# cambyse/po-rrt

Hardware: AMD Instinct MI355X
Metric: RRT node-expansions/sec on map_benchmark.pgm (higher is better)
Workload: dtype f64

## Files before the change

### po_rrt_amd/csrc/porrt_device.hpp

```cpp
#pragma once
#include <hip/hip_runtime.h>
#include <stdint.h>
#include <string>
#include <vector>
#include "../../include/porrt_hip.h"

namespace porrt {

template <int NEV>
struct ScopedEvents {
    hipEvent_t e[NEV];
    ScopedEvents() { for (int i = 0; i < NEV; ++i) e[i] = nullptr; }
    hipError_t create() {
        for (int i = 0; i < NEV; ++i) { const hipError_t r = hipEventCreate(&e[i]); if (r != hipSuccess) return r; }
        return hipSuccess;
    }
    ~ScopedEvents() { for (int i = 0; i < NEV; ++i) if (e[i]) (void)hipEventDestroy(e[i]); }
    ScopedEvents(const ScopedEvents &) = delete;
    ScopedEvents &operator=(const ScopedEvents &) = delete;
};

template <class Launch, class GoingOn>
static int sweep_to_fixpoint(hipStream_t stream, uint32_t *flags, size_t rows, int cur, Launch &&launch, GoingOn &&going_on, const char *who,
                             uint64_t &sweeps, std::string &err) {
// ... 91 lines not shown
#else
#define PORRT_T0() do {} while (0)
#define PORRT_TACC(rc, slot) do {} while (0)
#endif
#ifndef PORRT_TIMING_FROM
#define PORRT_TIMING_FROM 0
#endif
#ifndef PORRT_TIMING_UNTIL
#define PORRT_TIMING_UNTIL 0x7FFFFFFF
#endif
#if defined(PORRT_TIMING) && PORRT_TIMING == 1
#define PORRT_TACC_A(rc, slot) do { if (b >= (uint32_t)PORRT_TIMING_FROM && b < (uint32_t)PORRT_TIMING_UNTIL) PORRT_TACC(rc, slot); else t__0 = wall_clock64(); } while (0)
#define PORRT_TACC_B(rc, slot) do { (void)t__0; } while (0)
#elif defined(PORRT_TIMING)
#define PORRT_TACC_A(rc, slot) do { (void)t__0; } while (0)
#define PORRT_TACC_B(rc, slot) do { if (b >= (uint32_t)PORRT_TIMING_FROM && b < (uint32_t)PORRT_TIMING_UNTIL) PORRT_TACC(rc, slot); else t__0 = wall_clock64(); } while (0)
#else
#define PORRT_TACC_A(rc, slot) do {} while (0)
#define PORRT_TACC_B(rc, slot) do {} while (0)
#endif
#if defined(PORRT_TIMING) && PORRT_TIMING == 3
#undef PORRT_TACC_B
#define PORRT_TACC_B(rc, slot) do { (void)t__0; } while (0)
#define PORRT_TACC_C(rc, slot) PORRT_TACC(rc, slot)
#elif defined(PORRT_TIMING)
#define PORRT_TACC_C(rc, slot) do { (void)t__0; } while (0)
#else
#define PORRT_TACC_C(rc, slot) do {} while (0)
#endif

#if defined(PORRT_TIMING) && PORRT_TIMING == 4
#undef PORRT_TACC_B
#define PORRT_TACC_B(rc, slot) do { (void)t__0; } while (0)
#define PORRT_TACC_H(rc, slot) do { if (b >= (uint32_t)PORRT_TIMING_FROM && b < (uint32_t)PORRT_TIMING_UNTIL) PORRT_TACC(rc, slot); else t__0 = wall_clock64(); } while (0)
#define PORRT_TACC_S(rc, slot) do { if (TeamT::kSize == 64 && b >= (uint32_t)PORRT_TIMING_FROM && b < (uint32_t)PORRT_TIMING_UNTIL) PORRT_TACC(rc, slot); else t__0 = wall_clock64(); } while (0)
#elif defined(PORRT_TIMING)
#define PORRT_TACC_H(rc, slot) do { (void)t__0; } while (0)
#define PORRT_TACC_S(rc, slot) PORRT_TACC_B(rc, slot)
#else
#define PORRT_TACC_H(rc, slot) do {} while (0)
#define PORRT_TACC_S(rc, slot) do {} while (0)
#endif
#if defined(PORRT_TIMING) && PORRT_TIMING == 5
#undef PORRT_TACC_B
#define PORRT_TACC_B(rc, slot) do { (void)t__0; } while (0)
#endif

struct BestCost {
    unsigned long long cost_bits;
    uint32_t final_id, path_len, overflow, pad;
};

typedef float flt2 __attribute__((ext_vector_type(2)));
struct RunConst {
    double *nx, *ny;
    int *rep;
    flt2 *rep_f;
    double bx0, by0, binv_w, binv_h;
    uint32_t *rg_cnt;
    unsigned long long *rg_occ;
    uint32_t *rg_dir;
    double *pg_xy;
    int *pg_id;
    double *pg_d;
    uint32_t *slot_of;
    uint32_t rg_maxp, pg_cap;
    double *distA, *distB;
    int *parent;
    unsigned long long *reachA, *reachB;
    uint8_t *vid;
    uint8_t *final_flag;
    unsigned long long *final_mask;
    uint32_t *n_at;
    unsigned long long *valid_mask;
    Counters *cnt;
    double *sx, *sy;
    uint32_t *sworld;
    const double *inj_xy;
    unsigned long long inj_base, inj_n;
    double *q_x, *q_y;
    double *kq_x, *kq_y;
    int *kq_vid;
    int *q_nn;
    int *q_vid;
    uint32_t *cand_cnt;
    int *cand_id;
    double *cand_val;
    double *cand_xy;
    uint32_t cand_cap;
    uint32_t cand_K;
    const double *rad_T2;
    uint32_t *e_from, *e_to, *e_tv;
    uint32_t e_cap;
    KdRec *kd_rec;
    KdBox *kd_box;
    KdBox *loc_box;
    uint32_t loc_stride;
    KdMove *kd_losers;
    int *pend_new, *pend_pool;
    uint32_t *pend_off, *pend_n, *pend_cur, *pend_state;
    uint32_t pend_cap, pool_cap;
    int *bc_scratch;
    uint32_t bc_cap;
    uint32_t *bc_cursor;
    BestCost *bc_out;
    unsigned long long *kd_hint;
// ... 1 lines not shown
    uint32_t *kd_depth;
    uint32_t *kd_gexit;
    int *loc_cur;
    uint32_t *loc_dcur, *loc_gex, *loc_flags, *g_nd;
    double *g_nd_x, *g_nd_y;
    KdBox *g_nd_box;
    int *g_id;
    double *g_x, *g_y;
    uint32_t g_cap;
    uint32_t *g_snap;
    double gp_x, gp_y;
    const uint8_t *cls;
    const uint32_t *sat;
    const uint8_t *clr;
    uint32_t W, H;
    double low0, low1, ppm;
    int domain, has_grid;
    int n_validities;
    unsigned long long validities[65];
    unsigned long long all_worlds;
    int goal_kind;
    uint32_t G;
    double gcx[64], gcy[64];
    unsigned long long gmask[64];
    double g_l1;
    double w2g_x[64], w2g_y[64];
    double zone_x, zone_y, visibility;
    double s_low0, s_low1, s_up0, s_up1;
    double max_step;
    int mode;
    uint16_t *perm;
    double *ssx, *ssy;
    double *bq_x, *bq_y;
    uint16_t *bq_k;
    double *t2_at;
    uint32_t tile_R;
    uint32_t part_stride;
    uint32_t q_stride;
    double start_x, start_y;
    unsigned long long root_reach;
    int root_vid;
    unsigned long long rng_st_lo, rng_st_hi, rng_inc_lo, rng_inc_hi;
    struct PcgJump *jump;
    RunConst *self;
    uint32_t *zero0;
    unsigned long long zero_words;
    uint32_t *sched_i0, *sched_nb;
    uint32_t sched_min, sched_max, sched_K, sched_steps;
    uint32_t sched_max_nodes;
    uint32_t cand_par3;
    uint32_t hint_max;
    uint32_t kd_lazy;
};

#define GPTR(T) T __attribute__((address_space(1))) *
template <class T>
__device__ __forceinline__ GPTR(T) as_global(T *p) { return (GPTR(T))(uintptr_t)p; }
template <class T>
__device__ __forceinline__ GPTR(const T) as_global(const T *p) { return (GPTR(const T))(uintptr_t)p; }
template <class T>
__device__ __forceinline__ T g_atomic_add(GPTR(T) p, T v) { return __hip_atomic_fetch_add(p, v, __ATOMIC_RELAXED, __HIP_MEMORY_SCOPE_AGENT); }
template <class T>
__device__ __forceinline__ T g_atomic_or(GPTR(T) p, T v) { return __hip_atomic_fetch_or(p, v, __ATOMIC_RELAXED, __HIP_MEMORY_SCOPE_AGENT); }
template <class T>
__device__ __forceinline__ T g_atomic_min(GPTR(T) p, T v) { return __hip_atomic_fetch_min(p, v, __ATOMIC_RELAXED, __HIP_MEMORY_SCOPE_AGENT); }

__device__ __forceinline__ uint32_t uni(uint32_t v) { return (uint32_t)__builtin_amdgcn_readfirstlane((int)v); }
__device__ __forceinline__ double uni_d(double v) {
    const unsigned long long b = (unsigned long long)__double_as_longlong(v);
    const unsigned long long lo = uni((uint32_t)b), hi = uni((uint32_t)(b >> 32));
    return __longlong_as_double((long long)(lo | (hi << 32)));
}

#ifndef PORRT_RC_SCALAR
#define PORRT_RC_SCALAR 1
#endif
__device__ __forceinline__ const RunConst &rc_const(const RunConst *p) {
#if PORRT_RC_SCALAR
    const uintptr_t a = (uintptr_t)p;
    const uintptr_t u = (uintptr_t)uni((uint32_t)a) | ((uintptr_t)uni((uint32_t)(a >> 32)) << 32);
    return *(const RunConst *)(const RunConst __attribute__((address_space(4))) *)u;
#else
    return *p;
#endif
}
__device__ __forceinline__ const RunConst &rc_const(const RunConst &rc) { return rc_const(&rc); }

__device__ __forceinline__ uint32_t row_nb(const RunConst &rc, uint32_t b, uint32_t nb_arg) {
    return rc.sched_nb ? ((GPTR(const uint32_t))(uintptr_t)rc.sched_nb)[b] : nb_arg;
}
__device__ __forceinline__ uint32_t row_i0(const RunConst &rc, uint32_t b, uint32_t i0_arg) {
    return rc.sched_i0 ? ((GPTR(const uint32_t))(uintptr_t)rc.sched_i0)[b] : i0_arg;
}


__device__ __forceinline__ uint32_t q_off(const RunConst &rc, uint32_t b) { return (b & 1u) * rc.q_stride; }
__device__ __forceinline__ uint32_t cand_slot(const RunConst &rc, uint32_t b) { return rc.cand_par3 ? b % 3u : (b & 1u); }
__device__ __forceinline__ size_t cand_off(const RunConst &rc, uint32_t b, uint32_t k) { return ((size_t)cand_slot(rc, b) * rc.cand_K + k) * rc.cand_cap; }
__device__ __forceinline__ uint32_t cand_cnt_at(const RunConst &rc, uint32_t b, uint32_t k) { return cand_slot(rc, b) * rc.cand_K + k; }
__device__ __forceinline__ size_t cand_val_off(const RunConst &rc, uint32_t b, uint32_t k) {
    return rc.cand_par3 ? ((size_t)cand_slot(rc, b) * rc.cand_K + k) * rc.cand_cap : (size_t)k * rc.cand_cap;
}
__device__ __forceinline__ uint32_t cand_count(const RunConst &rc, uint32_t b, uint32_t k) {
    const uint32_t c = as_global(rc.cand_cnt)[cand_cnt_at(rc, b, k)];
    return c < rc.cand_cap ? c : rc.cand_cap;
}
__device__ __forceinline__ unsigned long long f64_bits(double d) { return (unsigned long long)__double_as_longlong(d); }

__device__ __forceinline__ uint32_t f64_as_u32(double v) {
    if (!(v == v)) return 0u;
    if (v <= 0.0) return 0u;
    if (v >= 4294967295.0) return 4294967295u;
    return (uint32_t)v;
}

__device__ __forceinline__ void to_pixel(const RunConst &rc, double x, double y, uint32_t &i, uint32_t &j) {
    double t = (y - rc.low1) * rc.ppm;
    i = f64_as_u32((double)(rc.H - 1) - t);
    j = f64_as_u32((x - rc.low0) * rc.ppm);
}

__device__ __forceinline__ double dist2(double ax, double ay, double bx, double by) {
    double dx = bx - ax, dy = by - ay;
    double xx = dx * dx, yy = dy * dy;
    return xx + yy;
}

__device__ __forceinline__ void wave_first_min(double &value, uint32_t &pos) {
    constexpr uint32_t kNone = 0xFFFFFFFFu;
    for (uint32_t s = 32; s >= 1; s >>= 1) {
        const double oc = __shfl_xor(value, (int)s);
        const uint32_t op = (uint32_t)__shfl_xor((int)pos, (int)s);
        if (op != kNone && (pos == kNone || oc < value || (oc == value && op < pos))) { value = oc; pos = op; }
    }
}

__device__ __forceinline__ void oct_to(int o, int x, int y, int &ox, int &oy) {
    switch (o) {
    case 0: ox = x; oy = y; break;
// ... 77 lines not shown
    const int fb = (o == 1 || o == 6) ? 1 : ((o == 2 || o == 5) ? -1 : 0);
    const int fc = (o == 1 || o == 2) ? 1 : ((o == 5 || o == 6) ? -1 : 0);
    const int fd = (o == 0 || o == 3) ? 1 : ((o == 4 || o == 7) ? -1 : 0);
    constexpr int kRayChunk = Grid::kRayChunk;
    for (int x = sx, y = sy; x <= ex;) {
        int c[kRayChunk];
        const int n = ex - x + 1 < kRayChunk ? ex - x + 1 : kRayChunk;
#pragma unroll
        for (int u = 0; u < kRayChunk; ++u) {
            c[u] = CLS_FREE;
            if (u < n) {
                const int pi = fa * x + fb * y, pj = fc * x + fd * y;
                c[u] = grid.at((uint32_t)pi, (uint32_t)pj);
                if (e >= 0) { y += 1; e -= ddx; }
                e += ddy;
                ++x;
            }
        }
#pragma unroll
        for (int u = 0; u < kRayChunk; ++u) {
            if (u >= n) break;
            if (rc.domain == 0) {
                if (c[u] == CLS_HIGH0) return CLS_HIGH;
                worst = c[u] > worst ? c[u] : worst;
            } else if (c[u] != CLS_FREE) {
                if (c[u] == CLS_HIGH || c[u] == CLS_HIGH0) return CLS_HIGH;
                if (c[u] == CLS_BAD) { *err |= ERR_RASTER; return CLS_HIGH; }
                if (worst >= CLS_ZONE && worst != c[u]) { *err |= ERR_RASTER; return CLS_HIGH; }
                worst = c[u];
            }
        }
    }
    return worst;
}
template <class Grid>
__device__ __forceinline__ int traversed_class(const RunConst &rc, const Grid &grid, double ax, double ay, double bx, double by, uint32_t *err) {
    uint32_t ai, aj, bi, bj;
    to_pixel(rc, ax, ay, ai, aj);
    to_pixel(rc, bx, by, bi, bj);
    return traversed_class_px(rc, grid, ai, aj, bi, bj, err);
}

__device__ __forceinline__ bool segment_in_clearance(uint32_t ai, uint32_t aj, uint32_t bi, uint32_t bj, uint32_t clr_b) {
    const uint32_t di = ai > bi ? ai - bi : bi - ai, dj = aj > bj ? aj - bj : bj - aj;
    return (di > dj ? di : dj) < clr_b;
}

__device__ __forceinline__ int state_class(const RunConst &rc, double x, double y, uint32_t *err) {
    uint32_t i, j;
    to_pixel(rc, x, y, i, j);
    if (i >= rc.H || j >= rc.W) { *err |= ERR_RASTER; return CLS_HIGH; }
    int c = as_global(rc.cls)[i * rc.W + j];
    if (c == CLS_BAD) { *err |= ERR_RASTER; return CLS_HIGH; }
    return c == CLS_HIGH0 ? CLS_HIGH : c;
}

__device__ __forceinline__ int class_to_validity(const RunConst &rc, int cls) {
    if (cls == CLS_FREE) return rc.n_validities - 1;
    if (cls >= CLS_ZONE) return cls - CLS_ZONE;
    return -1;
}

template <class Grid>
__device__ bool goal_hit(const RunConst &rc, const Grid &grid, double x, double y, unsigned long long &mask, uint32_t *err) {
    if (rc.goal_kind == 1) {
        for (uint32_t g = 0; g < rc.G; ++g) {
            double d = fabs(rc.gcx[g] - x);
            d += fabs(rc.gcy[g] - y);
            if (d < rc.g_l1) { mask = rc.gmask[g]; return true; }
        }
        return false;
    }
    if (rc.goal_kind == 2) {
        double D = sqrt(dist2(x, y, rc.zone_x, rc.zone_y));
        if (D < rc.visibility) {
            int c = traversed_class(rc, grid, x, y, rc.zone_x, rc.zone_y, err);
            if (c != CLS_HIGH) { mask = 1ull; return true; }
        }
    }
    return false;
}

typedef unsigned __int128 u128;
__device__ __forceinline__ u128 mk128(unsigned long long lo, unsigned long long hi) { return ((u128)hi << 64) | lo; }

struct PcgJump {
    unsigned long long mult_lo[64], mult_hi[64], plus_lo[64], plus_hi[64];
};

__device__ __forceinline__ unsigned long long pcg_output(u128 s) {
    uint32_t rot = (uint32_t)(s >> 122);
    unsigned long long xsl = (unsigned long long)(s >> 64) ^ (unsigned long long)s;
    return (xsl >> rot) | (xsl << ((64 - rot) & 63));
}

__device__ __forceinline__ double gen_range_once(unsigned long long r, double low, double high, bool *retry) {
    double v12 = __longlong_as_double((long long)((r >> 12) | 0x3FF0000000000000ull));
    double v01 = v12 - 1.0;
    double scale = high - low;
    double prod = v01 * scale;
    double res = prod + low;
    if (!(res < high)) *retry = true;
    return res;
}

__global__ void k_gen_samples(const RunConst *__restrict__ rcp, const PcgJump *__restrict__ jt, unsigned long long it0,
// ... 560 lines not shown
        as_global(rc.pg_id)[(size_t)page * kPage + (slot % kPage)] = (int)nid;
        as_global(rc.slot_of)[nid] = page * kPage + (slot % kPage);
        if (!GROUP || rc.q_stride) {
            as_global(rc.nx)[nid] = x[q];
            as_global(rc.ny)[nid] = y[q];
        }
    }
#pragma unroll
    for (uint32_t h = 0; h < RPT; ++h) {
        const uint32_t r = tid + h * T;
        if (r < kRegions) rg_new[r] = s_old[r] + s_add[r];
    }
    if (tid < kOccWords) {
        unsigned long long w = 0;
        for (uint32_t i = 0; i < 64u; ++i) {
            const uint32_t r = tid * 64u + i;
            if (r < kRegions && s_old[r] + s_add[r] > 0u) w |= 1ull << i;
        }
        as_global(rc.rg_occ)[((b + 1u) & 1u) * kOccWords + tid] = w;
    }
    if (tid == 0) { as_global(rc.t2_at)[b + 1] = t2_next; rc.cnt->n_pages += s_misc[0]; }
}

__device__ __forceinline__ uint32_t rank_before(const RunConst &rc, uint32_t b, uint32_t vwords, uint32_t k) {
    uint32_t r = 0;
    auto vm = as_global(rc.valid_mask) + (size_t)b * vwords;
    for (uint32_t w = 0; w < (k >> 6); ++w) r += __popcll(vm[w]);
    r += __popcll(vm[k >> 6] & ((1ull << (k & 63u)) - 1ull));
    return r;
}
template <int CTRL>
__device__ __forceinline__ uint32_t dpp_u32(uint32_t v) { return (uint32_t)__builtin_amdgcn_update_dpp((int)v, (int)v, CTRL, 0xF, 0xF, false); }
template <int CTRL>
__device__ __forceinline__ double dpp_f64(double v) {
    const unsigned long long b = (unsigned long long)__double_as_longlong(v);
    const unsigned long long lo = dpp_u32<CTRL>((uint32_t)b), hi = dpp_u32<CTRL>((uint32_t)(b >> 32));
    return __longlong_as_double((long long)(lo | (hi << 32)));
}
constexpr int kDppRowRor = 0x120;
constexpr int kDppRowBcast = 0x150;
#ifndef PORRT_DPP
#define PORRT_DPP 1
#endif

__device__ __forceinline__ uint32_t rank_before_lanes(const RunConst &rc, uint32_t b, uint32_t vwords, uint32_t k, uint32_t lane, uint32_t stride) {
    auto vm = as_global(rc.valid_mask) + (size_t)b * vwords;
    const uint32_t wk = k >> 6;
    uint32_t r = 0;
    for (uint32_t w0 = 0; w0 <= wk; w0 += stride) {
        const uint32_t w = w0 + lane;
        unsigned long long v = w <= wk ? vm[w] : 0ull;
        if (w == wk) v &= (1ull << (k & 63u)) - 1ull;
        r += (uint32_t)__popcll(v);
    }
    if (PORRT_DPP && stride == 16u) {
        r += dpp_u32<kDppRowRor + 8>(r); r += dpp_u32<kDppRowRor + 4>(r); r += dpp_u32<kDppRowRor + 2>(r); r += dpp_u32<kDppRowRor + 1>(r);
        return r;
    }
    for (uint32_t off = stride >> 1; off > 0; off >>= 1) r += (uint32_t)__shfl_xor((int)r, (int)off);
    return r;
}

__device__ __forceinline__ TileGrid load_tile(const RunConst &rc, uint8_t *tile, double px, double py, uint32_t lane, uint32_t stride) {
    TileGrid g;
    g.lds = tile; g.glob = rc.cls; g.W = rc.W; g.TW = 2u * rc.tile_R + 1u;
    uint32_t ci, cj;
    to_pixel(rc, px, py, ci, cj);
    g.oi = (int)ci - (int)rc.tile_R;
    g.oj = (int)cj - (int)rc.tile_R;
    const uint32_t n = g.TW * g.TW;
    for (uint32_t t = lane; t < n; t += stride) {
        const uint32_t ri = t / g.TW, rj = t - ri * g.TW;
        const int i = g.oi + (int)ri, j = g.oj + (int)rj;
        uint8_t c = CLS_BAD;
        if (i >= 0 && j >= 0 && (uint32_t)i < rc.H && (uint32_t)j < rc.W) c = as_global(rc.cls)[(uint32_t)i * rc.W + (uint32_t)j];
        tile[t] = c;
    }
    return g;
}

template <class T>
__device__ __forceinline__ T wave_min_u(T v) {
    for (int off = 32; off > 0; off >>= 1) {
        T o = __shfl_xor(v, off);
        v = o < v ? o : v;
    }
    return v;
}
__device__ __forceinline__ uint32_t wave_sum(uint32_t v) {
    for (int off = 32; off > 0; off >>= 1) v += __shfl_xor(v, off);
    return v;
}
__device__ __forceinline__ unsigned long long wave_or(unsigned long long v) {
    for (int off = 32; off > 0; off >>= 1) v |= __shfl_xor(v, off);
    return v;
}

__device__ __forceinline__ bool kd_left(double x, double y, double wx, double wy, uint32_t depth) {
    return (depth & 1u) ? (y < wy) : (x < wx);
}

__device__ bool kd_preorder_less(const RunConst &rc, int u, int v) {
    const uint32_t gu = as_global(rc.kd_gexit)[u], gv = as_global(rc.kd_gexit)[v];
    const bool ou = gu & kOnG, ov = gv & kOnG;
    const uint32_t iu = gu & ~kOnG, iv = gv & ~kOnG;
    if (ou && ov) return iu < iv;
// ... 2097 lines not shown
```

### po_rrt_amd/csrc/porrt_group.hpp

```cpp
#pragma once
#include "porrt_device.hpp"
#include "porrt_span.hpp"

namespace porrt {


template <int GL, int R, bool WITHD, class Visit>
__device__ __forceinline__ void gscan_disc(const RunConst &rc, uint32_t b, const GTeam<GL> &tm, double qx, double qy, double rho, uint32_t N, Visit visit,
                                           uint32_t skip_region = 0xFFFFFFFFu) {
    const uint32_t gl = tm.gl;
    int cx0, cy0, cx1, cy1;
    rep_cell(rc, qx - rho, qy - rho, kRG, cx0, cy0);
    rep_cell(rc, qx + rho, qy + rho, kRG, cx1, cy1);
    const uint32_t x0 = (uint32_t)cx0, y0 = (uint32_t)cy0;
    const uint32_t w = (uint32_t)(cx1 - cx0 + 1), nreg = w * (uint32_t)(cy1 - cy0 + 1);
    constexpr int U = (int)kPage / GL;
    if (nreg * 16u > N) {
#if !PORRT_PAGE_LOADS
        auto gx = as_global(rc.nx), gy = as_global(rc.ny), gdA = as_global(rc.distA);
#endif
        for (uint32_t j0 = 0; j0 < N; j0 += (uint32_t)(U * GL)) {
            double x[U], y[U], d[U];
#pragma unroll
            for (int u = 0; u < U; ++u) {
                const uint32_t j = j0 + (uint32_t)(GL * u) + gl;
#if PORRT_PAGE_LOADS
                const uint32_t o = (j < N ? j : 0u) * 8u;
                x[u] = g_at(rc.nx, o);
                y[u] = g_at(rc.ny, o);
                d[u] = WITHD ? g_at(rc.distA, o) : 0.0;
#else
                x[u] = gx[j < N ? j : 0u];
                y[u] = gy[j < N ? j : 0u];
                d[u] = WITHD ? gdA[j < N ? j : 0u] : 0.0;
#endif
            }
#pragma unroll
            for (int u = 0; u < U; ++u)
                if (j0 + (uint32_t)(GL * u) < N) visit(x[u], y[u], d[u], (int)(j0 + (uint32_t)(GL * u) + gl), j0 + (uint32_t)(GL * u) + gl < N);
        }
        return;
    }
    auto gcnt = as_global(rc.rg_cnt) + (b & 1u) * kRegions;
    auto gdir = as_global(rc.rg_dir);
#if PORRT_PAGE_LOADS
    const PageBuf pb = page_buf(rc);
#else
    auto gxy = as_global(reinterpret_cast<const dbl2 *>(rc.pg_xy));
    auto gid = as_global(rc.pg_id);
    auto gpd = as_global(rc.pg_d);
#endif
    for (uint32_t r0 = 0; r0 < nreg; r0 += (uint32_t)GL) {
        const uint32_t r = r0 + gl;
        uint32_t reg = 0, cnt = 0;
        if (r < nreg) {
            const uint32_t ry = r / w;
            reg = (y0 + ry) * kRG + x0 + (r - ry * w);
            cnt = reg == skip_region ? 0u : gcnt[reg];
        }
        uint32_t page = reg;
        for (uint32_t lvl = 0;; ++lvl) {
            const uint32_t have = cnt > lvl * kPage ? cnt - lvl * kPage : 0u;
            unsigned long long m = tm.ballot(have > 0u);
            if (!m) break;
            uint32_t page_next = 0;
            if (have > kPage) page_next = gdir[(size_t)reg * rc.rg_maxp + lvl + 1u];
            while (m) {
                uint32_t pg[R], pc[R];
#pragma unroll
                for (int q = 0; q < R; ++q) {
                    pg[q] = 0; pc[q] = 0;
                    if (m) {
                        const int l = (int)__builtin_ctzll(m);
                        m &= m - 1;
                        pg[q] = tm.shfl(page, l);
                        const uint32_t h = tm.shfl(have, l);
                        pc[q] = h < kPage ? h : kPage;
                    }
                }
                dbl2 v[R][U];
                double d[R][U];
                int id[R][U];
#pragma unroll
                for (int q = 0; q < R; ++q)
#pragma unroll
                    for (int u = 0; u < U; ++u) {
                        const uint32_t sl = (uint32_t)(u * GL) + gl;
                        const bool ld = sl < pc[q];
#if PORRT_PAGE_LOADS
                        const uint32_t at = ld ? pg[q] * kPage + sl : kNoSlot;
                        v[q][u] = page_xy(pb, at);
                        id[q][u] = page_id(pb, at);
                        d[q][u] = WITHD ? page_d(pb, at) : 0.0;
#else
                        v[q][u] = ld ? gxy[(size_t)pg[q] * kPage + sl] : dbl2{0.0, 0.0};
                        id[q][u] = ld ? gid[(size_t)pg[q] * kPage + sl] : -1;
                        d[q][u] = (WITHD && ld) ? gpd[(size_t)pg[q] * kPage + sl] : 0.0;
#endif
                    }
#if PORRT_PAGE_LOADS
                __atomic_signal_fence(__ATOMIC_SEQ_CST);
#endif
#pragma unroll
                for (int q = 0; q < R; ++q)
#pragma unroll
                    for (int u = 0; u < U; ++u)
                        if ((uint32_t)(u * GL) < pc[q]) visit(v[q][u].x, v[q][u].y, d[q][u], id[q][u], (uint32_t)(u * GL) + gl < pc[q]);
            }
            page = page_next;
        }
    }
}
// ... 390 lines not shown
#pragma unroll
        for (int u = 0; u < U; ++u) {
            if (!(via[u] >= 0.0) || f64_bits(via[u]) != f64_bits(dB[u])) continue;
#if PORRT_PAGE_LOADS
            auto gpar = g_ptr(rc.parent, (uint32_t)j[u] * 4u);
#else
            auto gpar = as_global(rc.parent) + j[u];
#endif
            int old = *gpar;
            while (old < N || id[u] < old) {
                int expect = old;
                if (__hip_atomic_compare_exchange_strong(gpar, &expect, id[u], __ATOMIC_RELAXED, __ATOMIC_RELAXED, __HIP_MEMORY_SCOPE_AGENT)) break;
                old = expect;
            }
#if PORRT_PAGE_LOADS
            *g_ptr(rc.distA, (uint32_t)j[u] * 8u) = via[u];
            *g_ptr(rc.pg_d, g_at(rc.slot_of, (uint32_t)j[u] * 4u) * 8u) = via[u];
#else
            gdA[j[u]] = via[u];
            gpd[gso[j[u]]] = via[u];
#endif
        }
    }
}

#ifndef PORRT_NN2_WAVES
#define PORRT_NN2_WAVES 5
#endif
template <int GL, int WV = 4>
__global__ __launch_bounds__(WV * 64) __attribute__((amdgpu_waves_per_eu(PORRT_NN2_WAVES, 8))) void k_nn2(const RunConst *__restrict__ rcp, uint32_t b, uint32_t i0, uint32_t nb, uint32_t vwords, uint32_t cb,
                                             uint32_t cnb, uint32_t cflat) {
    static_assert(GL == 16 || GL == 32 || GL == 64, "group size");
    constexpr uint32_t SPB = (uint32_t)WV * 64u / GL;
    uint32_t bx = blockIdx.x, by = blockIdx.y;
    xcd_swizzle(bx, by);
    const RunConst &rc = rc_const(rcp + by);
    GTeam<GL> tm;
    tm.gl = threadIdx.x % GL;
    tm.base = (threadIdx.x & 63u) - tm.gl;
    const uint32_t near_blocks = (nb + SPB - 1u) / SPB;
    if (bx >= near_blocks) {
        if (cflat) {
            PORRT_T0();
            commit_flat_span<(uint32_t)WV * 64u>(rc, cb, vwords, cnb, bx - near_blocks);
            PORRT_TACC_A(rc, 4);
            return;
        }
        const uint32_t ck = (bx - near_blocks) * SPB + threadIdx.x / GL;
        PORRT_T0();
        if (ck < cnb && ck < row_nb(rc, cb, cnb)) commit_rrt_sample(rc, cb, vwords, ck, tm.gl, GL);
        PORRT_TACC_A(rc, 4);
        return;
    }
    const uint32_t slot = bx * SPB + threadIdx.x / GL;
    if (slot >= row_nb(rc, b, nb)) return;
    PORRT_T0();
    const size_t so = (size_t)b * rc.part_stride + slot;
    const uint32_t k = as_global(rc.perm)[so];
    const uint32_t N = as_global(rc.n_at)[b];
    const double sqx = as_global(rc.ssx)[so], sqy = as_global(rc.ssy)[so];
    (void)i0;
    int nn = -1;
    double fx = 0.0, fy = 0.0;
    bool easy = false;
    const double lim = 0.7 * rc.max_step, t2b = as_global(rc.t2_at)[b];
    const double lim2 = lim * lim < t2b ? lim * lim : t2b;
    uint32_t err = 0;
    int cls_own = CLS_FREE;
    if (rc.has_grid) cls_own = state_class(rc, sqx, sqy, &err);
    const double perr = 1.3e-7 * (fabs(sqx) + fabs(sqy) + 2.0 * lim);
    const double limf = lim - perr, limf2 = limf > 0.0 ? (limf * limf < t2b ? limf * limf : t2b * (1.0 - 1e-6)) : -1.0;
    (void)lim2;
    for (int l = 0; l < 2 && !easy; ++l) {
        int cx, cy;
        const int G = rep_dim(l);
        rep_cell(rc, sqx, sqy, G, cx, cy);
        bool near = false;
        if (tm.gl < 9u) {
            const int x = cx + (int)(tm.gl % 3u) - 1, y = cy + (int)(tm.gl / 3u) - 1;
            if (x >= 0 && y >= 0 && x < G && y < G) {
                const flt2 pf = as_global(rc.rep_f)[rep_off(l) + y * G + x];
                near = dist2((double)pf.x, (double)pf.y, sqx, sqy) <= limf2;
            }
        }
        easy = tm.ballot(near) != 0ull;
    }
    PORRT_TACC_A(rc, 0);
    if (!easy) group_nn<GL>(rc, b, tm, N, sqx, sqy, nn, fx, fy);
    PORRT_TACC_A(rc, 1);
    double tx = sqx, ty = sqy;
    if (!easy) {
        double step = fabs(tx - fx);
        step += fabs(ty - fy);
        if (step > rc.max_step) {
            const double lambda = rc.max_step / step;
            double ux = (tx - fx) * lambda, uy = (ty - fy) * lambda;
            tx = fx + ux;
            ty = fy + uy;
        }
    }
    bool valid = true;
    if (rc.has_grid) {
        int cls = cls_own;
        if (tx != sqx || ty != sqy) { err = 0; cls = state_class(rc, tx, ty, &err); }
        valid = cls == CLS_FREE && !err;
    }
    PORRT_TACC_A(rc, 2);
    if (tm.gl == 0) {
        as_global(rc.q_x)[k] = tx;
        as_global(rc.q_y)[k] = ty;
        const size_t o2 = (size_t)b * rc.part_stride + k;
        as_global(rc.kq_x)[o2] = tx; as_global(rc.kq_y)[o2] = ty; as_global(rc.kq_vid)[o2] = valid ? 0 : -1;
        as_global(rc.q_nn)[k] = nn;
        int qv = valid ? 0 : -1;
        if (valid && rc.goal_kind != 0 && tx == rc.gp_x && ty == rc.gp_y) {
            const uint32_t slot = atomicAdd(&rc.cnt->clone_n, 1u);
            if (slot < 64u) { rc.cnt->clone_k[slot] = k; qv = 1; }
        }
        as_global(rc.q_vid)[k] = qv;
        as_global(rc.bq_x)[slot] = tx; as_global(rc.bq_y)[slot] = ty; as_global(rc.bq_k)[slot] = qv == 0 ? (uint16_t)k : (uint16_t)0xFFFFu;
        if (valid) atomicOr(&rc.valid_mask[(size_t)b * vwords + (k >> 6)], 1ull << (k & 63u));
        if (err) atomicOr(&rc.cnt->err, err);
    }
}

__host__ __device__ inline size_t conn2_lds_bytes(uint32_t GL) {
    (void)GL;
    return (64u / 16u) * kHitBytes;
}
static_assert(kInsertLds <= kFileLds && kGTrackLds <= kFileLds, "the filing's one-round-trip form is the largest of the riders' scratch areas");
__host__ __device__ inline size_t conn2_riders_lds_bytes() { return kFileLds; }
__host__ __device__ inline size_t conn2_wg4_lds_bytes(uint32_t GL) {
    const size_t a = 4u * conn2_lds_bytes(GL);
    static_assert(kGTrackLds <= 4u * (64u / 16u) * kHitBytes, "g_track_step uses the same bytes");
    static_assert(kFileLds <= 4u * (64u / 16u) * kHitBytes, "file_step_fast uses the same bytes");
    return a > kInsertLds ? a : kInsertLds;
}

__device__ __forceinline__ void rider_file(const RunConst &rc, uint32_t b, uint32_t nb, uint32_t vwords, uint8_t *lds, uint32_t fast) {
    if (fast && nb <= 4u * 256u) file_step_fast<256u, 4u, true>(rc, b, nb, vwords, lds);
    else insert_step_pages<1>(rc, b, nb, vwords, lds);
}
__device__ __forceinline__ void rider_gtrack(const RunConst &rc, uint32_t b, uint32_t nb, uint32_t vwords, uint8_t *lds, uint32_t fast) {
    if (fast) g_track_step<2>(rc, b, nb, vwords, lds);
    else g_track_step<1>(rc, b, nb, vwords, lds);
}
#if defined(PORRT_TIMING) && PORRT_TIMING == 5
#define RIDERS_T0() const unsigned long long rt__0 = wall_clock64(); const uint32_t rt__w = b < 8u ? 0u : ((rc.cnt->g_first_dup[0] & rc.cnt->g_first_dup[1]) != 0xFFFFFFFFu ? 2u : 1u)
#define RIDERS_MARK(role)                                                                                          \
    do {                                                                                                           \
        __syncthreads();                                                                                           \
        if (threadIdx.x == 0) { atomicAdd(&rc.cnt->tim[3u * (role) + rt__w], wall_clock64() - rt__0); if ((role) == 0u) atomicAdd(&rc.cnt->tim[9u + rt__w], 1ull); } \
    } while (0)
#else
#define RIDERS_T0() do {} while (0)
#define RIDERS_MARK(role) do {} while (0)
#endif

template <int GL>
__device__ __attribute__((noinline)) int group_nn_call(const RunConst &rc_arg, uint32_t b, uint32_t gl, uint32_t base, uint32_t N, double px, double py) {
// ... 155 lines not shown
#else
    uint32_t &err = err_out;
#endif
    const uint32_t lane = threadIdx.x & 63u;
    constexpr uint32_t kWaveHits = (64u / (uint32_t)GL) * (kLdsHits * (uint32_t)(GL / 16));
    Team<1> tw;
    tw.scr_d = nullptr; tw.scr_i = nullptr; tw.wave = 0; tw.lane = lane;
    TableGrid grid;
    grid.p = rc.cls; grid.W = rc.W;
    const uint32_t cap = rc.cand_cap;
    const MemHits Mh = mem_hits(rc, b, kh);
    PORRT_T0();
    if (toth <= kWaveHits) {
        LdsHits Wl;
        Wl.hx = (LdsPtr<double>)wb;
        Wl.hy = Wl.hx + kWaveHits;
        Wl.hd = Wl.hy + kWaveHits;
        Wl.hid = (LdsPtr<int>)(Wl.hd + kWaveHits);
        Wl.out_id = Mh.out_id; Wl.out_val = Mh.out_val; Wl.out_cnt = Mh.out_cnt; Wl.out_cap = Mh.out_cap;
        for (uint32_t a0 = 0; a0 < toth; a0 += 256u) {
            int jd[4];
            dbl2 v[4];
            double d[4];
#pragma unroll
            for (uint32_t u = 0; u < 4u; ++u) {
                const uint32_t a = a0 + u * 64u + lane;
                jd[u] = a < toth ? Mh.sid[a] : 0;
                v[u] = a < toth ? Mh.sxy[a] : dbl2{0.0, 0.0};
                d[u] = a < toth ? Mh.sd[a] : 0.0;
            }
#pragma unroll
            for (uint32_t u = 0; u < 4u; ++u) {
                const uint32_t a = a0 + u * 64u + lane;
                if (a < toth) { Wl.hid[a] = jd[u]; Wl.hx[a] = v[u].x; Wl.hy[a] = v[u].y; Wl.hd[a] = d[u]; }
            }
        }
        __builtin_amdgcn_wave_barrier();
        PORRT_TACC_H(rc, 0);
        connect_rrt_sample(rc, tw, Wl, grid, b, kh, idh, pxh, pyh, toth, err, nullptr, 0, clrh, [&]() { return wave_nn(rc, b, N, pxh, pyh); });
        __builtin_amdgcn_wave_barrier();
        PORRT_TACC_H(rc, 3);
    } else {
        connect_rrt_sample(rc, tw, Mh, grid, b, kh, idh, pxh, pyh, toth < cap ? toth : cap, err, nullptr, 0, clrh,
                           [&]() { return wave_nn(rc, b, N, pxh, pyh); });
    }
#if PORRT_PAGE_LOADS
    if (err) err_out |= err;
#endif
}

#ifndef PORRT_CONN2_WAVES
#define PORRT_CONN2_WAVES 4
#endif
template <int GL>
__device__ __forceinline__ void conn2_wave(const RunConst &rc, uint32_t b, uint32_t vwords, uint32_t N, double T2, uint32_t k, double px, double py, uint8_t *wl) {
    const uint32_t lane = threadIdx.x & 63u;
    GTeam<GL> tm;
    tm.gl = threadIdx.x % GL;
    tm.base = lane - tm.gl;
    const bool act = k != 0xFFFFu;
    uint32_t err = 0;
    PORRT_T0();
    uint32_t id = 0, tot = 0;
    int clr_b = 0;
    bool heavy = false;
    const uint32_t cap = rc.cand_cap;
    TableGrid grid;
    grid.p = rc.cls; grid.W = rc.W;
    if (act) {
        id = N + rank_before_lanes(rc, b, vwords, k, tm.gl, (uint32_t)GL);
        if (rc.has_grid) {
            uint32_t bi, bj;
            to_pixel(rc, px, py, bi, bj);
            if (bi < rc.H && bj < rc.W) clr_b = as_global(rc.clr)[bi * rc.W + bj];
        }
        constexpr uint32_t kHits = kLdsHits * (uint32_t)(GL / 16);
        uint8_t *hb = wl + (lane / (uint32_t)GL) * (kHits * 28u);
        LdsHits L;
        L.hx = (LdsPtr<double>)hb;
        L.hy = L.hx + kHits;
        L.hd = L.hy + kHits;
        L.hid = (LdsPtr<int>)(L.hd + kHits);
        const MemHits M = mem_hits(rc, b, k);
        L.out_id = M.out_id; L.out_val = M.out_val; L.out_cnt = M.out_cnt; L.out_cap = M.out_cap;
        PORRT_TACC_B(rc, 0);
        gscan_disc<GL, 1, true>(rc, b, tm, px, py, disc_radius(T2, px, py), N, [&](double x, double y, double dA, int jd, bool ok) {
            const bool in = ok && dist2(x, y, px, py) <= T2;
            const unsigned long long hm = tm.ballot(in);
            const uint32_t pos = tot + (uint32_t)__popcll(hm & ((1ull << tm.gl) - 1ull));
            if (in) {
                if (pos < kHits) { L.hid[pos] = jd; L.hx[pos] = x; L.hy[pos] = y; L.hd[pos] = dA; }
                else if (pos < cap) { M.sid[pos] = jd; dbl2 v; v.x = x; v.y = y; M.sxy[pos] = v; M.sd[pos] = dA; }
                else err |= (uint32_t)ERR_CAND_OVERFLOW;
            }
            tot += (uint32_t)__popcll(hm);
        });
        __builtin_amdgcn_wave_barrier();
        PORRT_TACC_B(rc, 1);
        if (tot <= kHits) {
            connect_rrt_sample(rc, tm, L, grid, b, k, id, px, py, tot, err, nullptr, 0, clr_b,
                               [&]() { return group_nn_call<GL>(rc, b, tm.gl, tm.base, N, px, py); });
            PORRT_TACC_B(rc, 2);
        } else {
            heavy = true;
            if (tm.gl == 0) atomicAdd(&rc.cnt->n_heavy, 1u);
            for (uint32_t a = tm.gl; a < kHits; a += (uint32_t)GL) {
                M.sid[a] = L.hid[a];
                dbl2 v;
                v.x = L.hx[a]; v.y = L.hy[a];
                M.sxy[a] = v;
                M.sd[a] = L.hd[a];
            }
        }
    }
    unsigned long long hv = __ballot(heavy && tm.gl == 0);
    if (hv) {
        __builtin_amdgcn_s_waitcnt(0x0F70);
        __builtin_amdgcn_wave_barrier();
        while (hv) {
            const int l = (int)__builtin_ctzll(hv);
            hv &= hv - 1;
            const uint32_t kh = uni((uint32_t)__shfl((int)k, l)), idh = uni((uint32_t)__shfl((int)id, l)), toth = uni((uint32_t)__shfl((int)tot, l));
            const int clrh = (int)uni((uint32_t)__shfl(clr_b, l));
            const double pxh = uni_d(__shfl(px, l)), pyh = uni_d(__shfl(py, l));
            heavy_sample_wave<GL>(rc, b, N, kh, idh, toth, clrh, pxh, pyh, wl, err);
        }
        PORRT_TACC_B(rc, 3);
    }
    if (err) atomicOr(&rc.cnt->err, err);
}

template <int GL>
__global__ __launch_bounds__(64) __attribute__((amdgpu_waves_per_eu(PORRT_CONN2_WAVES, 8))) void k_conn2(const RunConst *__restrict__ rcp, uint32_t b, uint32_t nb, uint32_t vwords) {
    static_assert(GL == 16 || GL == 32 || GL == 64, "group size");
    constexpr uint32_t SPB = 64u / GL;
    extern __shared__ __attribute__((aligned(16))) uint8_t lds_dyn[];
    uint32_t bx = blockIdx.x, by = blockIdx.y;
    xcd_swizzle(bx, by);
    const RunConst &rc = rc_const(rcp + by);
    nb = row_nb(rc, b, nb);
    const uint32_t slot = bx * SPB + threadIdx.x / GL;
    if (bx * SPB >= nb) return;
    const uint32_t N = as_global(rc.n_at)[b];
    const double T2 = as_global(rc.t2_at)[b];
    uint32_t k = 0xFFFFu;
    double px = 0.0, py = 0.0;
    if (slot < nb) { k = as_global(rc.bq_k)[slot]; px = as_global(rc.bq_x)[slot]; py = as_global(rc.bq_y)[slot]; }
    conn2_wave<GL>(rc, b, vwords, N, T2, k, px, py, lds_dyn);
}

__global__ __launch_bounds__(256) __attribute__((amdgpu_waves_per_eu(PORRT_CONN2_WAVES, 8))) void k_conn2_riders(const RunConst *__restrict__ rcp, uint32_t b, uint32_t nb, uint32_t vwords, uint32_t lazy,
                                                                                                                  uint32_t fast) {
    extern __shared__ __attribute__((aligned(16))) uint8_t lds_dyn[];
    const RunConst &rc = rc_const(rcp + blockIdx.y);
    const uint32_t role = blockIdx.x;
    nb = row_nb(rc, b, nb);
    if (nb == 0) return;
    RIDERS_T0();
    if (role == 0) rider_file(rc, b, nb, vwords, lds_dyn, fast);
    else if (lazy && role == 2u) rider_gtrack(rc, b, nb, vwords, lds_dyn, fast);
    else clone_workgroup(rc, b, vwords, as_global(rc.n_at)[b], as_global(rc.t2_at)[b], fast);
    RIDERS_MARK(role);
}

template <int GL>
__global__ __launch_bounds__(256) __attribute__((amdgpu_waves_per_eu(PORRT_CONN2_WAVES, 8))) void k_conn2_wg4(const RunConst *__restrict__ rcp, uint32_t b, uint32_t nb, uint32_t vwords, uint32_t lazy, uint32_t fast) {
    static_assert(GL == 16 || GL == 32 || GL == 64, "group size");
    constexpr uint32_t SPB = 256u / GL;
    extern __shared__ __attribute__((aligned(16))) uint8_t lds_dyn[];
    uint32_t bx = blockIdx.x, by = blockIdx.y;
    const uint32_t ns = lazy ? 3u : 2u;
    const uint32_t role = xcd_swizzle_roles(bx, by, ns);
    const RunConst &rc = rc_const(rcp + by);
    nb = row_nb(rc, b, nb);
    if (nb == 0) return;
    if (role == 0) { rider_file(rc, b, nb, vwords, lds_dyn, fast); return; }
    if (lazy && role == 2u) { rider_gtrack(rc, b, nb, vwords, lds_dyn, fast); return; }
    const uint32_t slot = bx * SPB + threadIdx.x / GL;
    const uint32_t N = as_global(rc.n_at)[b];
    const double T2 = as_global(rc.t2_at)[b];
    uint32_t k = 0xFFFFu;
    double px = 0.0, py = 0.0;
    if (role == ns && slot < nb) { k = as_global(rc.bq_k)[slot]; px = as_global(rc.bq_x)[slot]; py = as_global(rc.bq_y)[slot]; }
    if (role == 1) { clone_workgroup(rc, b, vwords, N, T2, fast); return; }
    conn2_wave<GL>(rc, b, vwords, N, T2, k, px, py, lds_dyn + (threadIdx.x >> 6) * conn2_lds_bytes(GL));
}

template <int GL>
__global__ __launch_bounds__(256) void k_commit2(const RunConst *__restrict__ rcp, uint32_t b, uint32_t nb, uint32_t vwords) {
    const RunConst &rc = rc_const(rcp + blockIdx.y);
    const uint32_t k = (blockIdx.x * 256u + threadIdx.x) / GL;
    if (k < nb && k < row_nb(rc, b, nb)) commit_rrt_sample(rc, b, vwords, k, threadIdx.x % GL, GL);
}
__global__ __launch_bounds__(256) __attribute__((amdgpu_waves_per_eu(8, 8))) void k_commit_flat(const RunConst *__restrict__ rcp, uint32_t b, uint32_t nb, uint32_t vwords) {
    commit_flat_span<256u>(rc_const(rcp + blockIdx.y), b, vwords, nb, blockIdx.x);
}

}
```

Baseline: 351.7 million.

## Reorder RunConst fields and hoist scalar loads to cut memory round trips

Reorders the RunConst struct so fields used by the nearest-neighbour and connect kernels sit together, and pins them into scalar registers with inline-asm holds so they arrive in a few batched scalar loads. In the nearest-neighbour step, the own-cell class lookup is split into an issue half and a finish half, overlapping it with the first rep-grid probe. In the connect wave, the valid-mask words and clearance byte are loaded early and the rank computation is deferred into a callback inside the disc scan, so those loads overlap the scan's first loads. This adds struct-layout coupling and more register pressure, and relies on compiler-barrier tricks that could change scheduling unpredictably.

```diff
diff --git a/po_rrt_amd/csrc/porrt_device.hpp b/po_rrt_amd/csrc/porrt_device.hpp
--- a/po_rrt_amd/csrc/porrt_device.hpp
+++ b/po_rrt_amd/csrc/porrt_device.hpp
@@ -167,6 +167,123 @@
 };
 
 typedef float flt2 __attribute__((ext_vector_type(2)));
+#ifndef PORRT_STEP_TRIPS
+#define PORRT_STEP_TRIPS 1
+#endif
+#ifndef PORRT_STEP_TRIPS_NN2
+#define PORRT_STEP_TRIPS_NN2 PORRT_STEP_TRIPS
+#endif
+#ifndef PORRT_STEP_TRIPS_CONN2
+#define PORRT_STEP_TRIPS_CONN2 PORRT_STEP_TRIPS
+#endif
+#if PORRT_STEP_TRIPS
+struct RunConst {
+    uint32_t *sched_nb, *sched_i0;
+    uint32_t *n_at;
+    double *t2_at;
+    uint16_t *perm;
+    double *ssx, *ssy;
+    uint32_t part_stride, q_stride;
+    double max_step;
+    int has_grid, domain;
+    uint32_t W, H;
+    double low0, low1, ppm;
+    const uint8_t *cls;
+    const uint8_t *clr;
+    double bx0, by0, binv_w, binv_h;
+    flt2 *rep_f;
+    int *rep;
+    uint32_t *rg_cnt;
+    unsigned long long *rg_occ;
+    uint32_t *rg_dir;
+    double *pg_xy;
+    int *pg_id;
+    double *pg_d;
+    uint32_t rg_maxp, pg_cap;
+    uint32_t *slot_of;
+    double *nx, *ny;
+    uint16_t *bq_k;
+    double *bq_x, *bq_y;
+    unsigned long long *valid_mask;
+    double *distA, *distB;
+    int *parent;
+    Counters *cnt;
+    uint32_t *cand_cnt;
+    int *cand_id;
+    double *cand_val;
+    double *cand_xy;
+    uint32_t cand_cap, cand_K;
+    uint32_t cand_par3, kd_lazy;
+    double *q_x, *q_y;
+    int *q_nn;
+    int *q_vid;
+    double *kq_x, *kq_y;
+    int *kq_vid;
+    int goal_kind;
+    uint32_t G;
+    double gp_x, gp_y;
+    double g_l1;
+    uint8_t *final_flag;
+    unsigned long long *final_mask;
+    const uint32_t *sat;
+    double zone_x, zone_y, visibility;
+    KdRec *kd_rec;
+    int *kd_up;
+    uint32_t *kd_depth;
+    uint32_t *kd_gexit;
+    int *pend_new, *pend_pool;
+    uint32_t *pend_off, *pend_n, *pend_cur, *pend_state;
+    uint32_t pend_cap, pool_cap;
+    double *g_x, *g_y;
+    int *g_id;
+    uint32_t *g_nd;
+    double *g_nd_x, *g_nd_y;
+    KdBox *g_nd_box;
+    uint32_t g_cap, tile_R;
+    const double *rad_T2;
+    unsigned long long *reachA, *reachB;
+    uint8_t *vid;
+    double *sx, *sy;
+    uint32_t *sworld;
+    const double *inj_xy;
+    unsigned long long inj_base, inj_n;
+    uint32_t *e_from, *e_to, *e_tv;
+    uint32_t e_cap;
+    uint32_t loc_stride;
+    KdBox *kd_box;
+    KdBox *loc_box;
+    KdMove *kd_losers;
+    int *bc_scratch;
+    uint32_t *bc_cursor;
+    BestCost *bc_out;
+    uint32_t bc_cap;
+    int mode;
+    unsigned long long *kd_hint;
+    int *loc_cur;
+    uint32_t *loc_dcur, *loc_gex, *loc_flags;
+    uint32_t *g_snap;
+    int n_validities;
+    int root_vid;
+    unsigned long long all_worlds;
+    double s_low0, s_low1, s_up0, s_up1;
+    double start_x, start_y;
+    unsigned long long root_reach;
+    unsigned long long rng_st_lo, rng_st_hi, rng_inc_lo, rng_inc_hi;
+    struct PcgJump *jump;
+    RunConst *self;
+    uint32_t *zero0;
+    unsigned long long zero_words;
+    uint32_t sched_min, sched_max, sched_K, sched_steps;
+    uint32_t sched_max_nodes;
+    uint32_t hint_max;
+    unsigned long long validities[65];
+    double gcx[64], gcy[64];
+    unsigned long long gmask[64];
+    double w2g_x[64], w2g_y[64];
+    unsigned long long pad_[6];
+};
+static_assert(sizeof(RunConst) % 64 == 0, "a row of an array of rows starts on a cache line");
+#else
 struct RunConst {
     double *nx, *ny;
     int *rep;
@@ -274,6 +391,7 @@
     uint32_t hint_max;
     uint32_t kd_lazy;
 };
+#endif
 
 #define GPTR(T) T __attribute__((address_space(1))) *
 template <class T>
@@ -307,6 +425,49 @@
 #endif
 }
 __device__ __forceinline__ const RunConst &rc_const(const RunConst &rc) { return rc_const(&rc); }
+
+template <class T>
+__device__ __forceinline__ auto rc_bits(T v) {
+    static_assert(sizeof(T) == 4 || sizeof(T) == 8, "a field of one or two registers");
+    if constexpr (sizeof(T) == 8) return __builtin_bit_cast(unsigned long long, v);
+    else return __builtin_bit_cast(uint32_t, v);
+}
+#define PORRT_HS1(a) "s"(::porrt::rc_bits(a))
+#define PORRT_HS2(a, ...) PORRT_HS1(a), PORRT_HS1(__VA_ARGS__)
+#define PORRT_HS3(a, ...) PORRT_HS1(a), PORRT_HS2(__VA_ARGS__)
+#define PORRT_HS4(a, ...) PORRT_HS1(a), PORRT_HS3(__VA_ARGS__)
+#define PORRT_HS5(a, ...) PORRT_HS1(a), PORRT_HS4(__VA_ARGS__)
+#define PORRT_HS6(a, ...) PORRT_HS1(a), PORRT_HS5(__VA_ARGS__)
+#define PORRT_HS7(a, ...) PORRT_HS1(a), PORRT_HS6(__VA_ARGS__)
+#define PORRT_HS8(a, ...) PORRT_HS1(a), PORRT_HS7(__VA_ARGS__)
+#define PORRT_HS9(a, ...) PORRT_HS1(a), PORRT_HS8(__VA_ARGS__)
+#define PORRT_HS10(a, ...) PORRT_HS1(a), PORRT_HS9(__VA_ARGS__)
+#define PORRT_HS11(a, ...) PORRT_HS1(a), PORRT_HS10(__VA_ARGS__)
+#define PORRT_HS12(a, ...) PORRT_HS1(a), PORRT_HS11(__VA_ARGS__)
+#define PORRT_HS13(a, ...) PORRT_HS1(a), PORRT_HS12(__VA_ARGS__)
+#define PORRT_HS14(a, ...) PORRT_HS1(a), PORRT_HS13(__VA_ARGS__)
+#define PORRT_HS15(a, ...) PORRT_HS1(a), PORRT_HS14(__VA_ARGS__)
+#define PORRT_HS16(a, ...) PORRT_HS1(a), PORRT_HS15(__VA_ARGS__)
+#define PORRT_HS17(a, ...) PORRT_HS1(a), PORRT_HS16(__VA_ARGS__)
+#define PORRT_HS18(a, ...) PORRT_HS1(a), PORRT_HS17(__VA_ARGS__)
+#define PORRT_HS19(a, ...) PORRT_HS1(a), PORRT_HS18(__VA_ARGS__)
+#define PORRT_HS20(a, ...) PORRT_HS1(a), PORRT_HS19(__VA_ARGS__)
+#define PORRT_HS21(a, ...) PORRT_HS1(a), PORRT_HS20(__VA_ARGS__)
+#define PORRT_HS22(a, ...) PORRT_HS1(a), PORRT_HS21(__VA_ARGS__)
+#define PORRT_HS23(a, ...) PORRT_HS1(a), PORRT_HS22(__VA_ARGS__)
+#define PORRT_HS24(a, ...) PORRT_HS1(a), PORRT_HS23(__VA_ARGS__)
+#define PORRT_HS25(a, ...) PORRT_HS1(a), PORRT_HS24(__VA_ARGS__)
+#define PORRT_HS26(a, ...) PORRT_HS1(a), PORRT_HS25(__VA_ARGS__)
+#define PORRT_HS27(a, ...) PORRT_HS1(a), PORRT_HS26(__VA_ARGS__)
+#define PORRT_HS28(a, ...) PORRT_HS1(a), PORRT_HS27(__VA_ARGS__)
+#define PORRT_HS_PICK(a1, a2, a3, a4, a5, a6, a7, a8, a9, a10, a11, a12, a13, a14, a15, a16, a17, a18, a19, a20, a21, a22, a23, a24, a25, a26, a27, a28, N, ...) \
+    PORRT_HS##N
+#if PORRT_STEP_TRIPS && PORRT_RC_SCALAR
+#define RC_HOLD(key, ...)                                                                                                                         \
+    asm("" : "+s"(key) : PORRT_HS_PICK(__VA_ARGS__, 28, 27, 26, 25, 24, 23, 22, 21, 20, 19, 18, 17, 16, 15, 14, 13, 12, 11, 10, 9, 8, 7, 6, 5, 4, 3, 2, 1)(__VA_ARGS__))
+#else
+#define RC_HOLD(key, ...) do {} while (0)
+#endif
 
 __device__ __forceinline__ uint32_t row_nb(const RunConst &rc, uint32_t b, uint32_t nb_arg) {
     return rc.sched_nb ? ((GPTR(const uint32_t))(uintptr_t)rc.sched_nb)[b] : nb_arg;
@@ -490,6 +651,16 @@
     if (i >= rc.H || j >= rc.W) { *err |= ERR_RASTER; return CLS_HIGH; }
     int c = as_global(rc.cls)[i * rc.W + j];
     if (c == CLS_BAD) { *err |= ERR_RASTER; return CLS_HIGH; }
+    return c == CLS_HIGH0 ? CLS_HIGH : c;
+}
+__device__ __forceinline__ int state_class_issue(const RunConst &rc, double x, double y, bool &inside) {
+    uint32_t i, j;
+    to_pixel(rc, x, y, i, j);
+    inside = i < rc.H && j < rc.W;
+    return as_global(rc.cls)[inside ? i * rc.W + j : 0u];
+}
+__device__ __forceinline__ int state_class_finish(int c, bool inside, uint32_t *err) {
+    if (!inside || c == CLS_BAD) { *err |= ERR_RASTER; return CLS_HIGH; }
     return c == CLS_HIGH0 ? CLS_HIGH : c;
 }
 
@@ -1156,6 +1327,25 @@
         unsigned long long v = w <= wk ? vm[w] : 0ull;
         if (w == wk) v &= (1ull << (k & 63u)) - 1ull;
         r += (uint32_t)__popcll(v);
+    }
+    if (PORRT_DPP && stride == 16u) {
+        r += dpp_u32<kDppRowRor + 8>(r); r += dpp_u32<kDppRowRor + 4>(r); r += dpp_u32<kDppRowRor + 2>(r); r += dpp_u32<kDppRowRor + 1>(r);
+        return r;
+    }
+    for (uint32_t off = stride >> 1; off > 0; off >>= 1) r += (uint32_t)__shfl_xor((int)r, (int)off);
+    return r;
+}
+
+template <uint32_t NW>
+__device__ __forceinline__ uint32_t rank_of_lane_words(const unsigned long long (&v)[NW], uint32_t k, uint32_t lane, uint32_t stride) {
+    const uint32_t wk = k >> 6;
+    uint32_t r = 0;
+#pragma unroll
+    for (uint32_t u = 0; u < NW; ++u) {
+        const uint32_t w = u * stride + lane;
+        unsigned long long x = w <= wk ? v[u] : 0ull;
+        if (w == wk) x &= (1ull << (k & 63u)) - 1ull;
+        r += (uint32_t)__popcll(x);
     }
     if (PORRT_DPP && stride == 16u) {
         r += dpp_u32<kDppRowRor + 8>(r); r += dpp_u32<kDppRowRor + 4>(r); r += dpp_u32<kDppRowRor + 2>(r); r += dpp_u32<kDppRowRor + 1>(r);
diff --git a/po_rrt_amd/csrc/porrt_group.hpp b/po_rrt_amd/csrc/porrt_group.hpp
--- a/po_rrt_amd/csrc/porrt_group.hpp
+++ b/po_rrt_amd/csrc/porrt_group.hpp
@@ -5,9 +5,10 @@
 namespace porrt {
 
 
-template <int GL, int R, bool WITHD, class Visit>
+struct GscanNothingBeside { __device__ __forceinline__ void operator()() const {} };
+template <int GL, int R, bool WITHD, class Visit, class Beside = GscanNothingBeside>
 __device__ __forceinline__ void gscan_disc(const RunConst &rc, uint32_t b, const GTeam<GL> &tm, double qx, double qy, double rho, uint32_t N, Visit visit,
-                                           uint32_t skip_region = 0xFFFFFFFFu) {
+                                           uint32_t skip_region = 0xFFFFFFFFu, Beside beside = Beside()) {
     const uint32_t gl = tm.gl;
     int cx0, cy0, cx1, cy1;
     rep_cell(rc, qx - rho, qy - rho, kRG, cx0, cy0);
@@ -19,6 +20,7 @@
 #if !PORRT_PAGE_LOADS
         auto gx = as_global(rc.nx), gy = as_global(rc.ny), gdA = as_global(rc.distA);
 #endif
+        beside();
         for (uint32_t j0 = 0; j0 < N; j0 += (uint32_t)(U * GL)) {
             double x[U], y[U], d[U];
 #pragma unroll
@@ -58,6 +60,7 @@
             reg = (y0 + ry) * kRG + x0 + (r - ry * w);
             cnt = reg == skip_region ? 0u : gcnt[reg];
         }
+        if (r0 == 0) beside();
         uint32_t page = reg;
         for (uint32_t lvl = 0;; ++lvl) {
             const uint32_t have = cnt > lvl * kPage ? cnt - lvl * kPage : 0u;
@@ -554,26 +557,56 @@
         PORRT_TACC_A(rc, 4);
         return;
     }
+    RC_HOLD(b, rc.sched_nb, rc.part_stride, rc.n_at, rc.t2_at, rc.perm, rc.ssx, rc.ssy, rc.max_step, rc.has_grid, rc.W, rc.H, rc.low0, rc.low1, rc.ppm,
+            rc.cls, rc.bx0, rc.by0, rc.binv_w, rc.binv_h, rc.rep_f);
     const uint32_t slot = bx * SPB + threadIdx.x / GL;
     if (slot >= row_nb(rc, b, nb)) return;
     PORRT_T0();
     const size_t so = (size_t)b * rc.part_stride + slot;
     const uint32_t k = as_global(rc.perm)[so];
+#if !PORRT_STEP_TRIPS_NN2
     const uint32_t N = as_global(rc.n_at)[b];
+#endif
     const double sqx = as_global(rc.ssx)[so], sqy = as_global(rc.ssy)[so];
     (void)i0;
     int nn = -1;
     double fx = 0.0, fy = 0.0;
     bool easy = false;
     const double lim = 0.7 * rc.max_step, t2b = as_global(rc.t2_at)[b];
+#if PORRT_STEP_TRIPS_NN2
+    __atomic_signal_fence(__ATOMIC_SEQ_CST);
+    const uint32_t N = as_global(rc.n_at)[b];
+#endif
     const double lim2 = lim * lim < t2b ? lim * lim : t2b;
     uint32_t err = 0;
     int cls_own = CLS_FREE;
+#if !PORRT_STEP_TRIPS_NN2
     if (rc.has_grid) cls_own = state_class(rc, sqx, sqy, &err);
+#endif
     const double perr = 1.3e-7 * (fabs(sqx) + fabs(sqy) + 2.0 * lim);
     const double limf = lim - perr, limf2 = limf > 0.0 ? (limf * limf < t2b ? limf * limf : t2b * (1.0 - 1e-6)) : -1.0;
     (void)lim2;
+#if PORRT_STEP_TRIPS_NN2
+    bool cls_in = false;
+    asm volatile("" ::"v"(sqx), "v"(sqy), "v"(t2b));
+    if (rc.has_grid) cls_own = state_class_issue(rc, sqx, sqy, cls_in);
+    {
+        int cx, cy;
+        const int G = rep_dim(0);
+        rep_cell(rc, sqx, sqy, G, cx, cy);
+        flt2 pf = {__builtin_nanf(""), __builtin_nanf("")};
+        if (tm.gl < 9u) {
+            const int x = cx + (int)(tm.gl % 3u) - 1, y = cy + (int)(tm.gl / 3u) - 1;
+            if (x >= 0 && y >= 0 && x < G && y < G) pf = as_global(rc.rep_f)[rep_off(0) + y * G + x];
+        }
+        __atomic_signal_fence(__ATOMIC_SEQ_CST);
+        if (rc.has_grid) cls_own = state_class_finish(cls_own, cls_in, &err);
+        easy = tm.ballot(dist2((double)pf.x, (double)pf.y, sqx, sqy) <= limf2) != 0ull;
+    }
+    for (int l = 1; l < 2 && !easy; ++l) {
+#else
     for (int l = 0; l < 2 && !easy; ++l) {
+#endif
         int cx, cy;
         const int G = rep_dim(l);
         rep_cell(rc, sqx, sqy, G, cx, cy);
@@ -608,6 +641,8 @@
         valid = cls == CLS_FREE && !err;
     }
     PORRT_TACC_A(rc, 2);
+    RC_HOLD(b, rc.q_x, rc.q_y, rc.kq_x, rc.kq_y, rc.kq_vid, rc.q_nn, rc.q_vid, rc.goal_kind, rc.gp_x, rc.gp_y, rc.bq_x, rc.bq_y, rc.bq_k, rc.valid_mask,
+            rc.cnt, rc.part_stride);
     if (tm.gl == 0) {
         as_global(rc.q_x)[k] = tx;
         as_global(rc.q_y)[k] = ty;
@@ -869,6 +904,9 @@
 #ifndef PORRT_CONN2_WAVES
 #define PORRT_CONN2_WAVES 4
 #endif
+#define CONN2_HOLD(rc, b)                                                                                                                          \
+    RC_HOLD(b, rc.sched_nb, rc.n_at, rc.t2_at, rc.bq_k, rc.bq_x, rc.bq_y, rc.valid_mask, rc.has_grid, rc.W, rc.H, rc.low0, rc.low1, rc.ppm, rc.clr,  \
+            rc.cand_cap, rc.bx0, rc.by0, rc.binv_w, rc.binv_h, rc.rg_cnt, rc.rg_dir, rc.rg_maxp, rc.pg_cap, rc.pg_xy, rc.pg_id, rc.pg_d)
 template <int GL>
 __device__ __forceinline__ void conn2_wave(const RunConst &rc, uint32_t b, uint32_t vwords, uint32_t N, double T2, uint32_t k, double px, double py, uint8_t *wl) {
     const uint32_t lane = threadIdx.x & 63u;
@@ -885,12 +923,41 @@
     TableGrid grid;
     grid.p = rc.cls; grid.W = rc.W;
     if (act) {
+#if PORRT_STEP_TRIPS_CONN2
+        asm("" : "+v"(px), "+v"(py));
+        constexpr uint32_t kVW = GL == 16 ? 2u : 1u;
+        const bool words_held = vwords <= kVW * (uint32_t)GL;
+        unsigned long long vw[kVW] = {};
+        if (words_held) {
+#pragma unroll
+            for (uint32_t u = 0; u < kVW; ++u) {
+                const uint32_t w = u * (uint32_t)GL + tm.gl;
+                vw[u] = w <= (k >> 6) ? as_global(rc.valid_mask)[(size_t)b * vwords + w] : 0ull;
+            }
+        } else {
+            id = N + rank_before_lanes(rc, b, vwords, k, tm.gl, (uint32_t)GL);
+        }
+        bool clr_in = false;
+        if (rc.has_grid) {
+            uint32_t bi, bj;
+            to_pixel(rc, px, py, bi, bj);
+            clr_in = bi < rc.H && bj < rc.W;
+            clr_b = as_global(rc.clr)[clr_in ? bi * rc.W + bj : 0u];
+        }
+        const auto beside = [&]() {
+            if constexpr (kVW == 2u) asm volatile("" : "+v"(vw[0]), "+v"(vw[1]), "+v"(clr_b)::"memory");
+            else asm volatile("" : "+v"(vw[0]), "+v"(clr_b)::"memory");
+            if (words_held) id = N + rank_of_lane_words(vw, k, tm.gl, (uint32_t)GL);
+            if (!clr_in) clr_b = 0;
+        };
+#else
         id = N + rank_before_lanes(rc, b, vwords, k, tm.gl, (uint32_t)GL);
         if (rc.has_grid) {
             uint32_t bi, bj;
             to_pixel(rc, px, py, bi, bj);
             if (bi < rc.H && bj < rc.W) clr_b = as_global(rc.clr)[bi * rc.W + bj];
         }
+#endif
         constexpr uint32_t kHits = kLdsHits * (uint32_t)(GL / 16);
         uint8_t *hb = wl + (lane / (uint32_t)GL) * (kHits * 28u);
         LdsHits L;
@@ -911,7 +978,11 @@
                 else err |= (uint32_t)ERR_CAND_OVERFLOW;
             }
             tot += (uint32_t)__popcll(hm);
+#if PORRT_STEP_TRIPS_CONN2
+        }, 0xFFFFFFFFu, beside);
+#else
         });
+#endif
         __builtin_amdgcn_wave_barrier();
         PORRT_TACC_B(rc, 1);
         if (tot <= kHits) {
@@ -955,6 +1026,7 @@
     uint32_t bx = blockIdx.x, by = blockIdx.y;
     xcd_swizzle(bx, by);
     const RunConst &rc = rc_const(rcp + by);
+    CONN2_HOLD(rc, b);
     nb = row_nb(rc, b, nb);
     const uint32_t slot = bx * SPB + threadIdx.x / GL;
     if (bx * SPB >= nb) return;
@@ -994,6 +1066,7 @@
     if (role == 0) { rider_file(rc, b, nb, vwords, lds_dyn, fast); return; }
     if (lazy && role == 2u) { rider_gtrack(rc, b, nb, vwords, lds_dyn, fast); return; }
     const uint32_t slot = bx * SPB + threadIdx.x / GL;
+    if (role == ns) CONN2_HOLD(rc, b);
     const uint32_t N = as_global(rc.n_at)[b];
     const double T2 = as_global(rc.t2_at)[b];
     uint32_t k = 0xFFFFu;
```

New measurement: 359.5 million (median of 6 runs). 2.2% higher.
